# thetengda/OKVIS2-X

Measured on AMD Instinct MI355X. Metric: Gauss-Newton iters/sec on 50-KF/2000-landmark window; ATE vs CPU ref, higher is better.
Workload: dtype f64; 1 GPU; 2048 independent S50 windows (50 KF / 2000 landmarks / 16000 reprojections, 49 IMU factors), DENSE_SCHUR + DOGLEG, all tolerances 0; windows_total=2048, windows_per_gpu=2048, parallelism=replicas x1 (one window batch per GPU, no collective in the loop)

## Files before the change

### okvis2-x_amd/csrc/jv_groups.hpp

```cpp
#pragma once
#include "device_problem.hpp"
#include "okvisgpu_math.hpp"

namespace okg {

static_assert(kLmGroupVisits == 256, "jvGroups runs as 256-thread workgroups of k_lm_backsub_jv");

__device__ __forceinline__ bool jvSelect(const DevProblem& P, int w) {
  const WinState& s = P.st[w];
  return !s.done && s.need_gn && !s.gn_failed;
}

__device__ __forceinline__ void jvAcc(double jc, double jg, double (&a)[3]) {
  a[0] += jc * jc;
  a[1] += jg * jg;
  a[2] += jc * jg;
}

__device__ __forceinline__ void jvGroups(const DevProblem& P, int block) {
  const int gid = (block * 256 + (int)threadIdx.x) >> 4, r = threadIdx.x & 15;
  const double* __restrict__ cF = P.vF;
  const double* __restrict__ yF = P.yF;
  int u = gid, w = 0, nr = 0, nb = 0, ld = 0;
  const double* J = nullptr;
  int off[4] = {-1, -1, -1, -1}, n[4] = {0, 0, 0, 0}, col[4] = {0, 0, 0, 0};
  double* out = nullptr;
  size_t ostride = 0;
  bool live = false;
  __shared__ double sVc[256 / 16][32][2];
  if (gid < P.n_fac) {
    const int f = gid, grp = threadIdx.x >> 4;
    const int fw = gmem(P.imu_win)[f], ffl = gmem(P.imu_flags)[f];
    const int4 blk = gmem(reinterpret_cast<const int4*>(P.imu_blocks))[f];
    const auto gst = gmem(P.st + fw);
    const int sDone = gst->done, sNeed = gst->need_gn, sFail = gst->gn_failed, lcur = gst->lcur;
    const int o0 = blk.x < 0 ? -1 : gmem(P.pose_f)[max(blk.x, 0)], o1 = blk.y < 0 ? -1 : gmem(P.sb_f)[max(blk.y, 0)],
              o2 = blk.z < 0 ? -1 : gmem(P.pose_f)[max(blk.z, 0)], o3 = blk.w < 0 ? -1 : gmem(P.sb_f)[max(blk.w, 0)];
    const int foff = gmem(P.win_foff)[fw];
    const bool fl = (sDone == 0) & (sNeed != 0) & (sFail == 0), act = fl & !(ffl & 2);
    double vcv[2], vgv[2];
#pragma unroll
    for (int h = 0; h < 2; ++h) {
      const int c = r + 16 * h;
      const int q = c < 6 ? 0 : c < 15 ? 1 : c < 21 ? 2 : 3;
      const int cq = c - (q == 0 ? 0 : q == 1 ? 6 : q == 2 ? 15 : 21);
      const int oq = q == 0 ? o0 : q == 1 ? o1 : q == 2 ? o2 : o3;
      const bool ok = act && c < 30 && oq >= 0;
      const size_t i = ok ? (size_t)foff + oq + cq : 0;
      const double sc = gmem(P.sF)[i], cv = gmem(cF)[i], yv = gmem(yF)[i];
      vcv[h] = ok ? sc * cv : 0.0;
      vgv[h] = ok ? -sc * yv : 0.0;
    }
    const auto Jr = gmem(pick2(lcur, P.imu_lin[0], P.imu_lin[1]) + (size_t)(act ? f : 0) * kImuLin + 15 +
                         30 * (size_t)min(r, 14));
    double jr[30];
#pragma unroll
    for (int c = 0; c < 30; ++c) jr[c] = Jr[c];
#pragma unroll
    for (int h = 0; h < 2; ++h) {
      sVc[grp][r + 16 * h][0] = vcv[h];
      sVc[grp][r + 16 * h][1] = vgv[h];
    }
    __builtin_amdgcn_fence(__ATOMIC_RELEASE, "wavefront");
    __builtin_amdgcn_wave_barrier();
    __builtin_amdgcn_fence(__ATOMIC_ACQUIRE, "wavefront");
    double jc0 = 0.0, jg0 = 0.0;
#pragma unroll
    for (int c = 0; c < 30; ++c) {
      jc0 += jr[c] * sVc[grp][c][0];
      jg0 += jr[c] * sVc[grp][c][1];
    }
    double a3[3] = {r < 15 ? jc0 * jc0 : 0.0, r < 15 ? jg0 * jg0 : 0.0, r < 15 ? jc0 * jg0 : 0.0};
#pragma unroll
    for (int k = 0; k < 3; ++k)
#pragma unroll
      for (int m = 8; m > 0; m >>= 1) a3[k] += __shfl_xor(a3[k], m, 64);
    if (fl && r == 0)
      for (int k = 0; k < 3; ++k) P.imu_jv[(size_t)k * P.n_fac + f] = a3[k];
    return;
  }
  if (u < P.n_fac) {
  } else if ((u -= P.n_fac) < P.n_pprior) {
    w = P.pp_win[u];
    if (jvSelect(P, w)) {
      live = true;
      out = P.pp_jv + u;
      ostride = P.n_pprior;
      J = P.pp_lin[P.st[w].lcur] + 42 * (size_t)u + 6;
      nr = 6; ld = 6; nb = 1;
      off[0] = P.pose_f[P.pp_block[u]]; n[0] = 6;
    }
  } else if ((u -= P.n_pprior) < P.n_sbprior) {
    w = P.sbp_win[u];
    if (jvSelect(P, w)) {
      live = true;
      out = P.sbp_jv + u;
      ostride = P.n_sbprior;
      J = P.sbp_lin[P.st[w].lcur] + 90 * (size_t)u + 9;
      nr = 9; ld = 9; nb = 1;
      off[0] = P.sb_f[P.sbp_block[u]]; n[0] = 9;
    }
  } else if ((u -= P.n_sbprior) < P.n_relpose) {
    w = P.rp_win[u];
    if (jvSelect(P, w)) {
      live = true;
      out = P.rp_jv + u;
      ostride = P.n_relpose;
      if (!(P.rp_flags[u] & 2)) {
        J = P.rp_lin[P.st[w].lcur] + kRelPoseLin * (size_t)u + 6;
        nr = 6; ld = 12; nb = 2;
        off[0] = P.pose_f[P.rp_blocks[2 * u]]; off[1] = P.pose_f[P.rp_blocks[2 * u + 1]];
        n[0] = 6; n[1] = 6; col[1] = 6;
// ... 30 lines not shown
```

### okvis2-x_amd/csrc/kernels_backsub.hip

```cpp
#include "device_problem.hpp"
#include "jv_groups.hpp"
#include "launch.hpp"
#include "okvisgpu_math.hpp"

namespace okg {

struct ExtTerm {
  double Je[12], ce[6], ge[6];
};
__device__ __forceinline__ bool loadExtTerm(const DevProblem& P, int o, int w, int xs, const double C_WS[9],
                                            const double p3[3], double w4, const double A[6], ExtTerm& X) {
  if (!(P.obs_flags[o] & 4)) return false;
  const int e = P.cam_pose[P.obs_cam[o]];
  const size_t b = (size_t)P.win_foff[w] + P.pose_f[e];
  extrJacobian(A, C_WS, p3, w4, P.pose[xs] + 7 * (size_t)e, X.Je);
#pragma unroll
  for (int c = 0; c < 6; ++c) {
    const double sc = P.sF[b + c];
    X.ce[c] = sc * P.vF[b + c];
    X.ge[c] = -sc * P.yF[b + c];
  }
  return true;
}

template <bool EXT>
__global__ __launch_bounds__(kLmGroupVisits) void k_lm_backsub_jv(const DevProblem* __restrict__ Pp) {
  const DevProblem& P = *Pp;
  if (!EXT && (int)blockIdx.x >= P.n_lmg) {
    jvGroups(P, (int)blockIdx.x - P.n_lmg);
    return;
  }
  const int t = threadIdx.x;
  const auto gi = gmem(reinterpret_cast<const int4*>(P.lmg_info + kLmgInfo * blockIdx.x));
  const int4 gi0 = gi[0], gi1 = gi[kLmgInfo / 4];
  const int l0 = gi0.x, l1 = gi1.x;
  const int w = gi0.z;
  const int v0 = gi0.y, v1 = gi1.y;
  const int v = v0 + t;
  const bool hasV = v < v1;
  const int vc = hasV ? v : v0;
  const int vLm = gmem(P.visit_lm)[vc], vPose = gmem(P.visit_pose)[vc];
  const int obB = gmem(P.visit_obs_begin)[vc], obE = gmem(P.visit_obs_begin)[vc + 1];
  const auto gst = gmem(P.st + w);
  const int sDone = gst->done, sNeed = gst->need_gn, sFail = gst->gn_failed, sLcur = gst->lcur, sXcur = gst->xcur;
  const bool skip = (sDone != 0) | (sNeed == 0) | (sFail != 0) | (((vLm ^ vPose ^ obB ^ obE) & (vc >> 31)) != 0);
  if (skip) return;
  __shared__ double sQ[3][kLmGroupVisits];
  __shared__ double sC[6][kLmGroupMax];
  const int l = hasV ? vLm : l0;
  const int pose = hasV ? vPose : 0;
  const int ob0 = hasV ? obB : 0, ob1 = hasV ? obE : 0;
  const auto lin = gmem(pick2(sLcur, P.obs_lin[0], P.obs_lin[1]));
  const int64_t S = P.obs_stride;
  const int lfreeI = gmem(P.lm_free)[l], pfI = gmem(P.pose_f)[pose];
  const auto hpp = gmem(pick2(sXcur, P.lm[0], P.lm[1]) + 4 * (size_t)l);
  const auto twp = gmem(pick2(sXcur, P.pose[0], P.pose[1]) + 7 * (size_t)pose);
  const double hp[4] = {hpp[0], hpp[1], hpp[2], hpp[3]};
  double tw[7];
#pragma unroll
  for (int k = 0; k < 7; ++k) tw[k] = (EXT || k < 3) ? twp[k] : 0.0;
  const int fl0 = gmem(P.obs_flags)[obB];
  double A0[6];
#pragma unroll
  for (int k = 0; k < 6; ++k) A0[k] = lin[(2 + k) * S + obB];
  asm volatile("" ::"v"(lfreeI), "v"(pfI), "v"(hp[0]), "v"(hp[1]), "v"(hp[2]), "v"(hp[3]), "v"(tw[0]), "v"(tw[1]),
               "v"(tw[2]), "v"(fl0), "v"(A0[0]), "v"(A0[1]), "v"(A0[2]), "v"(A0[3]), "v"(A0[4]), "v"(A0[5]));
  const int xs = sXcur;
  const int pf = hasV ? pfI : -1;
  const bool lfree = lfreeI != 0;
  double cp[6], gp[6];
  {
    const size_t b = pf >= 0 ? (size_t)P.win_foff[w] + pf : 0;
    const auto sFp = gmem(P.sF + b), vFp = gmem(P.vF + b), yFp = gmem(P.yF + b);
    double sc[6], vv[6], yy[6];
#pragma unroll
    for (int c = 0; c < 6; ++c) {
      sc[c] = sFp[c];
      vv[c] = vFp[c];
      yy[c] = yFp[c];
    }
#pragma unroll
    for (int c = 0; c < 6; ++c) {
      cp[c] = pf >= 0 ? sc[c] * vv[c] : 0.0;
      gp[c] = pf >= 0 ? -sc[c] * yy[c] : 0.0;
    }
  }
  const double w4 = hp[3];
  const double p3[3] = {hp[0] - tw[0] * w4, hp[1] - tw[1] * w4, hp[2] - tw[2] * w4};
  double C_WS[9];
  if (EXT) qrot(qnormalize(Q{tw[3], tw[4], tw[5], tw[6]}), C_WS);

  double q[3] = {0.0, 0.0, 0.0};
  if ((pf >= 0 || EXT) && lfree)
    for (int o = ob0; o < ob1; ++o) {
      double A[6], Jp[12], Jl[6];
      int fl = fl0;
#pragma unroll
      for (int k = 0; k < 6; ++k) A[k] = A0[k];
      if (o != ob0) {
        fl = gmem(P.obs_flags)[o];
#pragma unroll
        for (int k = 0; k < 6; ++k) A[k] = lin[(2 + k) * S + o];
      }
      const bool use = !(fl & 2);
#pragma unroll
      for (int k = 0; k < 6; ++k) A[k] = use ? A[k] : 0.0;
      obsJacobians(A, p3, w4, Jp, Jl);
      ExtTerm X;
      const bool hasE = EXT && loadExtTerm(P, o, w, xs, C_WS, p3, w4, A, X);
#pragma unroll
      for (int r = 0; r < 2; ++r) {
        double jg = 0.0;
#pragma unroll
        for (int c = 0; c < 6; ++c) jg += Jp[r * 6 + c] * gp[c];
        if (hasE)
#pragma unroll
          for (int c = 0; c < 6; ++c) jg += X.Je[r * 6 + c] * X.ge[c];
#pragma unroll
        for (int a = 0; a < 3; ++a) q[a] -= Jl[r * 3 + a] * jg;
      }
    }
#pragma unroll
  for (int a = 0; a < 3; ++a) sQ[a][t] = q[a];
  ldsBarrier();

  double lred[3] = {0.0, 0.0, 0.0};
  if (t < l1 - l0) {
    const int L = l0 + t;
    double c6[6] = {0.0, 0.0, 0.0, 0.0, 0.0, 0.0};
    const int lf = gmem(P.lm_free)[L];
    const int mb = gmem(P.lm_visit_begin)[L] - v0, me = gmem(P.lm_visit_begin)[L + 1] - v0;
    double li[9], s3[3], zz[3], dgv[3], lg[3];
#pragma unroll
    for (int i = 0; i < 9; ++i) li[i] = gmem(P.lm_Linv)[9 * (size_t)L + i];
#pragma unroll
    for (int a = 0; a < 3; ++a) {
      const size_t i = 3 * (size_t)L + a;
      s3[a] = gmem(P.sL)[i];
      zz[a] = gmem(P.lm_zz)[i];
      dgv[a] = gmem(P.diagL)[i];
      lg[a] = gmem(P.lm_g)[i];
    }
    if (lf) {
      double qs[3] = {0.0, 0.0, 0.0};
      for (int m = mb; m < me; ++m)
#pragma unroll
        for (int a = 0; a < 3; ++a) qs[a] += sQ[a][m];
      double u[3];
#pragma unroll
      for (int a = 0; a < 3; ++a) qs[a] *= s3[a];
#pragma unroll
      for (int a = 0; a < 3; ++a) u[a] = zz[a] - (li[a * 3] * qs[0] + li[a * 3 + 1] * qs[1] + li[a * 3 + 2] * qs[2]);
#pragma unroll
      for (int a = 0; a < 3; ++a) {
        double y = 0.0;
#pragma unroll
        for (int c = a; c < 3; ++c) y += li[c * 3 + a] * u[c];
        const size_t i = 3 * (size_t)L + a;
        const double dg = dgv[a];
        gmemw(P.yL)[i] = y;
        const double gn = -dg * y;
        gmemw(P.gnL)[i] = gn;
        const double gr = s3[a] * lg[a] / dg;
        const double vc = gr / dg;
        gmemw(P.dgL)[i] = gr;
        gmemw(P.vL)[i] = vc;
        lred[0] += gr * gr;
        lred[1] += gn * gn;
        lred[2] += gr * gn;
        c6[a] = s3[a] * vc;
        c6[3 + a] = -s3[a] * y;
      }
    }
#pragma unroll
    for (int i = 0; i < 6; ++i) sC[i][t] = c6[i];
  }
  ldsBarrier();

  const int u = hasV ? l - l0 : 0;
  double cl[3], gl[3];
#pragma unroll
  for (int c = 0; c < 3; ++c) {
    cl[c] = sC[c][u];
    gl[c] = sC[3 + c][u];
  }
  double acc[3] = {0.0, 0.0, 0.0};
  for (int o = ob0; o < ob1; ++o) {
    double A[6], Jp[12], Jl[6];
    const bool use = !(gmem(P.obs_flags)[o] & 2);
#pragma unroll
    for (int k = 0; k < 6; ++k) A[k] = lin[(2 + k) * S + o];
#pragma unroll
    for (int k = 0; k < 6; ++k) A[k] = use ? A[k] : 0.0;
    obsJacobians(A, p3, w4, Jp, Jl);
    ExtTerm X;
    const bool hasE = EXT && loadExtTerm(P, o, w, xs, C_WS, p3, w4, A, X);
#pragma unroll
    for (int r = 0; r < 2; ++r) {
      double jc = 0.0, jg = 0.0;
#pragma unroll
      for (int c = 0; c < 6; ++c) {
        jc += Jp[r * 6 + c] * cp[c];
        jg += Jp[r * 6 + c] * gp[c];
      }
      if (hasE)
#pragma unroll
        for (int c = 0; c < 6; ++c) {
          jc += X.Je[r * 6 + c] * X.ce[c];
          jg += X.Je[r * 6 + c] * X.ge[c];
        }
#pragma unroll
      for (int c = 0; c < 3; ++c) {
        jc += Jl[r * 3 + c] * cl[c];
        jg += Jl[r * 3 + c] * gl[c];
      }
      acc[0] += jc * jc;
      acc[1] += jg * jg;
      acc[2] += jc * jg;
    }
  }
  double red[6] = {acc[0], acc[1], acc[2], lred[0], lred[1], lred[2]};
#pragma unroll
  for (int k = 0; k < 6; ++k)
#pragma unroll
    for (int m = 32; m > 0; m >>= 1) red[k] += __shfl_xor(red[k], m, 64);
  __shared__ double sW[kLmGroupVisits / 64][6];
  if ((t & 63) == 0)
#pragma unroll
    for (int k = 0; k < 6; ++k) sW[t >> 6][k] = red[k];
  ldsBarrier();
  if (t < 6) {
    double a = sW[0][t];
#pragma unroll
    for (int wv = 1; wv < kLmGroupVisits / 64; ++wv) a += sW[wv][t];
    gmemw(P.grp_red)[(size_t)blockIdx.x * kGrpRed + t] = a;
  }
}

void launch_lm_backsub(const DevProblem& P, hipStream_t s) {
  if (P.n_xvisit > 0) {
    if (P.n_lmg > 0) hipLaunchKernelGGL(k_lm_backsub_jv<true>, dim3(P.n_lmg), dim3(kLmGroupVisits), 0, s, P.self);
    launch_jv(P, s);
    return;
  }
  const int nb = P.n_lmg + jvBlocks(P);
  if (nb > 0) hipLaunchKernelGGL(k_lm_backsub_jv<false>, dim3(nb), dim3(kLmGroupVisits), 0, s, P.self);
}

}
```

### okvis2-x_amd/csrc/kernels_control.hip

```cpp
#include <cfloat>

#include "block_reduce.hpp"
#include "dev_clock.hpp"
#include "device_problem.hpp"
#include "gradnorm.hpp"
#include "jv_groups.hpp"
#include "launch.hpp"
#include "okvisgpu_math.hpp"

namespace okg {

constexpr int kRBBatch = 256, kRBFew = 1024;

__device__ void finalizeIteration(const DevProblem& P, WinState& s) {
  if (s.done) return;
  if (s.iteration >= P.opt.max_num_iterations) {
    s.done = 1;
    s.termination = 1;
    return;
  }
  if (s.radius <= P.opt.min_radius) {
    s.done = 1;
    s.termination = 0;
  }
// ... 197 lines not shown
  DLCLK(0)
  const int foff = P.win_foff[w], fd = P.win_fdim[w];
  const int l0 = P.win_lm_range[2 * w], l1 = P.win_lm_range[2 * w + 1];
  double gg = 0.0, nn = 0.0, gn = 0.0;
  for (int e = t; e < fd; e += RB) {
    const double a = gmem(P.dgF)[foff + e], b = gmem(P.gnF)[foff + e];
    gg += a * a;
    nn += b * b;
    gn += a * b;
  }
  const int gb = P.win_lmg_range[2 * w], ge = P.win_lmg_range[2 * w + 1];
  for (int g = gb + t; g < ge; g += RB) {
    const auto r = gmem(P.grp_red + (size_t)g * kGrpRed);
    gg += r[3];
    nn += r[4];
    gn += r[5];
  }
  double alpha = s.alpha;
  if (sflagGn) {
    double r6[6];
    double a3[3];
    jvPartials(P, w, t, RB, a3);
    DLCLK(1)
    r6[0] = a3[0]; r6[1] = a3[1]; r6[2] = a3[2]; r6[3] = gg; r6[4] = nn; r6[5] = gn;
    blockSumN<RB, 6>(r6, sh);
    DLCLK(2)
    gg = r6[3];
    nn = r6[4];
    gn = r6[5];
    alpha = gg / r6[0];
    if (t == 0) {
      s.jcc = r6[0];
      s.jgg = r6[1];
      s.jcg = r6[2];
      s.alpha = alpha;
    }
  } else {
    double r3[3] = {gg, nn, gn};
    blockSumN<RB, 3>(r3, sh);
    gg = r3[0];
    nn = r3[1];
    gn = r3[2];
  }
  const double gradient_norm = sqrt(gg), gauss_newton_norm = sqrt(nn);
  const double radius = s.radius;
  double ca, cb;
  int dcase;
  if (gauss_newton_norm <= radius) {
    ca = 0.0; cb = 1.0; dcase = 1;
  } else if (gradient_norm * alpha >= radius) {
    ca = -(radius / gradient_norm); cb = 0.0; dcase = 2;
  } else {
    const double b_dot_a = -alpha * gn;
    const double a_squared_norm = (alpha * gradient_norm) * (alpha * gradient_norm);
    const double b_minus_a_squared_norm = a_squared_norm - 2 * b_dot_a + gauss_newton_norm * gauss_newton_norm;
    const double c = b_dot_a - a_squared_norm;
    const double d = sqrt(c * c + b_minus_a_squared_norm * (radius * radius - a_squared_norm));
    const double beta = (c <= 0) ? (d - c) / b_minus_a_squared_norm : (radius * radius - a_squared_norm) / (d + c);
    ca = -alpha * (1.0 - beta);
    cb = beta;
    dcase = 3;
  }
  const int xs = s.xcur, xd = 1 - s.xcur;
  double sn2 = 0.0, dn2 = 0.0, jr = 0.0;
  const int p0 = P.win_pose_range[2 * w], p1 = P.win_pose_range[2 * w + 1];
  for (int p = p0 + t; p < p1; p += RB) {
    const int pf = gmem(P.pose_f)[p];
    if (pf < 0) continue;
    double dg[6], gn[6], dia[6], sc[6], g[6], x[7];
    for (int c = 0; c < 6; ++c) {
      const size_t i = (size_t)foff + pf + c;
      dg[c] = gmem(P.dgF)[i];
      gn[c] = gmem(P.gnF)[i];
      dia[c] = gmem(P.diagF)[i];
      sc[c] = gmem(P.sF)[i];
      g[c] = gmem(P.gF)[i];
    }
    for (int k = 0; k < 7; ++k) x[k] = gmem(P.pose[xs])[7 * (size_t)p + k];
    double delta[6];
    for (int c = 0; c < 6; ++c) {
      const double v = ca * dg[c] + cb * gn[c];
      dn2 += v * v;
      const double st = v / dia[c];
      gmemw(P.stepF)[(size_t)foff + pf + c] = st;
      delta[c] = st * sc[c];
      jr += delta[c] * g[c];
    }
    const auto y = gmemw(P.pose[xd] + 7 * (size_t)p);
    const Q dq = deltaQ(delta[3], delta[4], delta[5]);
    const Q q = qnormalize(qmul(dq, qnormalize(Q{x[3], x[4], x[5], x[6]})));
    double yv[7] = {x[0] + delta[0], x[1] + delta[1], x[2] + delta[2], q.x, q.y, q.z, q.w};
    for (int k = 0; k < 7; ++k) {
      y[k] = yv[k];
      sn2 += (x[k] - yv[k]) * (x[k] - yv[k]);
    }
  }
  const int b0 = P.win_sb_range[2 * w], b1 = P.win_sb_range[2 * w + 1];
  for (int b = b0 + t; b < b1; b += RB) {
    const int sf = gmem(P.sb_f)[b];
    if (sf < 0) continue;
    const auto y = gmemw(P.sb[xd] + 9 * (size_t)b);
    double dg[9], gn[9], dia[9], sc[9], g[9], x[9];
    for (int c = 0; c < 9; ++c) {
      const size_t i = (size_t)foff + sf + c;
      dg[c] = gmem(P.dgF)[i];
      gn[c] = gmem(P.gnF)[i];
      dia[c] = gmem(P.diagF)[i];
      sc[c] = gmem(P.sF)[i];
      g[c] = gmem(P.gF)[i];
      x[c] = gmem(P.sb[xs])[9 * (size_t)b + c];
    }
    for (int c = 0; c < 9; ++c) {
      const double v = ca * dg[c] + cb * gn[c];
      dn2 += v * v;
      const double st = v / dia[c];
      gmemw(P.stepF)[(size_t)foff + sf + c] = st;
      jr += (st * sc[c]) * g[c];
      const double yv = x[c] + st * sc[c];
      y[c] = yv;
      sn2 += (x[c] - yv) * (x[c] - yv);
    }
  }
  DLCLK(3)
  struct LS { double x[4], dg[3], gn[3], dia[3], sl[3], g[3]; uint8_t f; };
  stridedBatched<RB, (RB >= 1024 ? 1 : 4)>(l0, l1,
                    [&](int l) {
                      LS v;
                      v.f = gmem(P.lm_free)[l];
                      for (int k = 0; k < 4; ++k) v.x[k] = gmem(P.lm[xs])[4 * (size_t)l + k];
                      for (int c = 0; c < 3; ++c) {
                        const size_t i = 3 * (size_t)l + c;
                        v.dg[c] = gmem(P.dgL)[i];
                        v.gn[c] = gmem(P.gnL)[i];
                        v.dia[c] = gmem(P.diagL)[i];
                        v.sl[c] = gmem(P.sL)[i];
                        v.g[c] = gmem(P.gL)[i];
                      }
                      return v;
                    },
                    [&](int l, const LS& v) {
                      if (!v.f) return;
                      const auto y = gmemw(P.lm[xd] + 4 * (size_t)l);
                      for (int c = 0; c < 3; ++c) {
                        const double vv = ca * v.dg[c] + cb * v.gn[c];
                        dn2 += vv * vv;
                        const double st = vv / v.dia[c];
                        gmemw(P.stepL)[3 * (size_t)l + c] = st;
                        jr += (st * v.sl[c]) * v.g[c];
                        const double yv = v.x[c] + st * v.sl[c];
                        y[c] = yv;
                        sn2 += (v.x[c] - yv) * (v.x[c] - yv);
                      }
                      y[3] = v.x[3];
                    });
  DLCLK(4)
  {
    double r3[3] = {sn2, dn2, jr};
    blockSumN<RB, 3>(r3, sh);
    sn2 = r3[0];
    dn2 = r3[1];
    jr = r3[2];
  }
  DLCLK(5)
  DLCLK_END
  if (t != 0) return;
  s.dogleg_step_norm = (dcase == 1) ? gauss_newton_norm : (dcase == 2) ? radius : sqrt(dn2);
  s.step_norm = sqrt(sn2);
  const double jj = (ca * ca) * s.jcc + 2.0 * (ca * cb) * s.jcg + (cb * cb) * s.jgg;
  s.model_cost_change = -(jr + 0.5 * jj);
  if (s.model_cost_change > 0.0) {
    s.step_valid = 1;
    s.consecutive_invalid = 0;
    s.eval_cand = 1;
  } else {
    s.step_valid = 0;
    s.eval_cand = 0;
    if (++s.consecutive_invalid >= P.opt.max_num_consecutive_invalid_steps) {
      s.done = 1;
      s.termination = 2;
      s.iteration -= 1;
      return;
    }
    s.num_unsucc += 1;
    s.mu *= 10.0;
    s.need_gn = 1;
    finalizeIteration(P, s);
  }
}

__global__ __launch_bounds__(256) void k_jv(const DevProblem* __restrict__ Pp) { jvGroups(*Pp, (int)blockIdx.x); }
void launch_jv(const DevProblem& P, hipStream_t s) {
  if (jvBlocks(P) > 0) hipLaunchKernelGGL(k_jv, dim3(jvBlocks(P)), dim3(256), 0, s, P.self);
}
void launch_reduce(const DevProblem& P, int mode, hipStream_t s) {
  if (P.few) hipLaunchKernelGGL(k_reduce<kRBFew>, dim3(P.n_win), dim3(kRBFew), 0, s, P.self, mode);
  else hipLaunchKernelGGL(k_reduce<kRBBatch>, dim3(P.n_win), dim3(kRBBatch), 0, s, P.self, mode);
}
void launch_gradnorm(const DevProblem& P, int lin_mode, hipStream_t s) {
  hipLaunchKernelGGL(k_gradnorm<kRBBatch>, dim3(P.n_win), dim3(kRBBatch), 0, s, P.self, lin_mode);
}
void launch_dogleg(const DevProblem& P, hipStream_t s) {
  if (P.few) hipLaunchKernelGGL(k_dogleg<kRBFew>, dim3(P.n_win), dim3(kRBFew), 0, s, P.self);
  else hipLaunchKernelGGL(k_dogleg<kRBBatch>, dim3(P.n_win), dim3(kRBBatch), 0, s, P.self);
}

__global__ __launch_bounds__(256) void k_select_current(const DevProblem* __restrict__ Pp) {
  const DevProblem& P = *Pp;
  const int w = blockIdx.x;
  if (P.st[w].xcur != 1) return;
  auto copy = [&](const int32_t* range, int stride, const double* src, double* dst) {
    const int64_t b = (int64_t)range[2 * w] * stride, e = (int64_t)range[2 * w + 1] * stride;
    for (int64_t i = b + threadIdx.x; i < e; i += blockDim.x) dst[i] = src[i];
  };
  copy(P.win_pose_range, 7, P.pose[1], P.pose[0]);
  copy(P.win_sb_range, 9, P.sb[1], P.sb[0]);
  copy(P.win_lm_range, 4, P.lm[1], P.lm[0]);
}

void launch_select_current(const DevProblem& P, hipStream_t s) {
  if (P.n_win > 0) hipLaunchKernelGGL(k_select_current, dim3(P.n_win), dim3(256), 0, s, P.self);
}

}
```

### okvis2-x_amd/csrc/launch.hpp

```cpp
#pragma once

#include <hip/hip_runtime.h>

#include "device_problem.hpp"

namespace okg {

void launch_eval(const DevProblem& P, int mode, hipStream_t s);
void launch_eval_few(const DevProblem& P, int mode, hipStream_t s);
void launch_eval_obs(const DevProblem& P, int mode, hipStream_t s);
void launch_eval_imu(const DevProblem& P, int mode, hipStream_t s);
void launch_eval_imu_as_solved(const DevProblem& P, int mode, hipStream_t s);
void launch_imu_append(const DevProblem& P, hipStream_t s);
struct ImuPropagateDev {
  int32_t n;
  double par[7];
  double* poses;
  double* sb;
  const int64_t* t_start;
  const int64_t* t_end;
  const int32_t* sbegin;
  const int64_t* ts;
  const double* ga;
  double* cov;
  double* jac;
  int32_t* steps;
};
void launch_imu_propagate(const ImuPropagateDev& A, hipStream_t s);
void launch_host_gather(const DevProblem& P, int mode, hipStream_t s);
void launch_host_scatter(const DevProblem& P, hipStream_t s);

void launch_lm_blocks(const DevProblem& P, int lin_mode, hipStream_t s);
void launch_imu_hess(const DevProblem& P, int lin_mode, hipStream_t s);
void launch_fgrad(const DevProblem& P, int lin_mode, hipStream_t s);
void launch_lm_prep(const DevProblem& P, hipStream_t s);
void launch_lin_few(const DevProblem& P, hipStream_t s);
void launch_zero_S(const DevProblem& P, hipStream_t s);
void launch_assemble(const DevProblem& P, hipStream_t s);
void launch_lm_backsub(const DevProblem& P, hipStream_t s);
void launch_assemble_gradnorm_few(const DevProblem& P, hipStream_t s);
void launch_assemble_pp(const DevProblem& P, hipStream_t s);
void launch_assemble_sb(const DevProblem& P, hipStream_t s);
void launch_lm_visit(const DevProblem& P, int mode, hipStream_t s);

size_t cholesky_persistent_lds();
size_t cholesky_pipe_lds();
void launch_cholesky(const DevProblem& P, hipStream_t s);
void launch_cholesky_pipe(const DevProblem& P, hipStream_t s, bool split);
void launch_cholesky_split_b(const DevProblem& P, hipStream_t s);

enum ReduceMode { R_COST_INIT = 0, R_COST_CAND = 1, R_JV = 2 };
void launch_reduce(const DevProblem& P, int mode, hipStream_t s);
void launch_jv(const DevProblem& P, hipStream_t s);
void launch_gradnorm(const DevProblem& P, int lin_mode, hipStream_t s);
void launch_dogleg(const DevProblem& P, hipStream_t s);
void launch_select_current(const DevProblem& P, hipStream_t s);

void launch_twopose_compute(const TwoPoseDev& T, hipStream_t s);
void launch_twopose_extr_compute(const TwoPoseExtrDev& T, hipStream_t s);
void launch_twopose_extr_eval(const TwoPoseExtrEvalDev& T, hipStream_t s);

void launch_match_prepare(const MatchDev& M, hipStream_t s);
void launch_match(const MatchDev& M, hipStream_t s);

constexpr uint8_t kLmInitialised = 1, kLmReset = 2, kLmNotInFront = 4;
void launch_update_landmarks(const DevProblem& P, double* quality, uint8_t* flags, double* obs_err, double* dirs,
                             hipStream_t s);

struct CovisWin {
  int32_t lm_begin, n_lm;
  int32_t pose_begin, n_state;
  int32_t word_begin, n_words;
  int32_t state_off, pad_;
  int64_t bits_off;
  int64_t counts_off;
};
constexpr size_t kCovisLdsBudget = 64 * 1024;
constexpr int kCovisTile = 32;
constexpr int kCovisChunk = 32;
constexpr int covisRowStride(int n_words) { return n_words | 1; }
constexpr size_t covisLdsBytes(int n_state, int n_words) { return 8 * (size_t)n_state * (size_t)covisRowStride(n_words); }
constexpr bool covisFitsLds(int n_state, int n_words) { return covisLdsBytes(n_state, n_words) <= kCovisLdsBudget; }
void launch_covis_bits(const DevProblem& P, const CovisWin* wins, int n_wins, const int32_t* word_rec, int n_words_total,
                       const uint8_t* excluded, unsigned long long* bits, hipStream_t s);
void launch_covis_counts(const CovisWin* wins, const int32_t* items0, int n0, size_t lds_bytes, const int32_t* items1,
                         int n1, const unsigned long long* bits, int32_t* counts, int32_t* n_observed, hipStream_t s);

}
```

### okvis2-x_amd/csrc/runtime.cpp

```cpp
#include <hip/hip_runtime.h>

#include <algorithm>
#include <chrono>
#include <cmath>
#include <condition_variable>
#include <cstdio>
#include <cstdlib>
#include <cstring>
#include <functional>
#include <map>
#include <memory>
#include <mutex>
#include <stdexcept>
#include <string>
#include <thread>
#include <vector>

#include "../../include/okvisgpu.h"
#include "device_problem.hpp"
#include "launch.hpp"
#include "loss.hpp"
#include "okvisgpu_math.hpp"
#include "plan.hpp"

// ... 1141 lines not shown
        continue;
      }
      iterStart = nowS();
      if (o->verbose) c->runTimed(c->phaseMs);
      else c->launchIterations(1);
      ++c->replays;
      st = c->readStates();
    }
    c->finish(st, sums);
    return (int)OKVISGPU_OK;
  });
}

static const char* kPhaseNames[OKVISGPU_N_PHASES] = {
    "lm_prep",     "zero_S",   "assemble",   "cholesky",  "lm_backsub", "gn_finalize",
    "jv",          "reduce_jv", "dogleg",   "eval_obs",
    "eval_imu",    "eval_priors", "reduce_cand", "lin_blocks", "gradnorm"};

const char* okvisgpu_phase_name(int32_t i) { return (i >= 0 && i < OKVISGPU_N_PHASES) ? kPhaseNames[i] : ""; }

int okvisgpu_profile_iteration(okvisgpu_ctx* c, double* ms) {
  if (!c || !ms) return OKVISGPU_ERR_INVALID_ARGUMENT;
  if (!c->inSolve) return fail(c, OKVISGPU_ERR_INVALID_ARGUMENT, "profile_iteration needs solve_begin");
  return guarded(c, [&]() {
    for (int i = 0; i < OKVISGPU_N_PHASES; ++i) ms[i] = 0.0;
    c->runTimed(ms);
    c->replays += 1;
    return (int)OKVISGPU_OK;
  });
}

namespace {
enum KernelId {
  K_ASSEMBLE_PP, K_ASSEMBLE_SB, K_CHOLESKY, K_LM_VISIT, K_LM_VISIT_PREP, K_EVAL_IMU, K_EVAL_OBS, K_JV,
  K_FGRAD, K_LM_BACKSUB, K_COUNT
};
const char* kKernelNames[K_COUNT] = {"k_assemble_pp", "k_assemble_sb", "k_cholesky", "k_lm_visit", "k_lm_visit_prep",
                                     "k_eval_imu",    "k_eval_obs",    "k_jv",       "k_fgrad",
                                     "k_lm_backsub_jv"};
const int kKernelBound[K_COUNT] = {0, 0, 1, 0, 0, 0, 0, 0, 0, 0};

double kernelWork(const HostBatch& B, const DevProblem& P, int k) {
  const double d8 = 8.0;
  const double nObs = P.n_obs, nVis = P.n_visit, nLm = P.n_lm, nImu = P.n_imu;
  switch (k) {
    case K_ASSEMBLE_PP: {
      double desc = 0, pairs = 0;
      for (const auto* list : {&B.asm_pp_items, &B.asm_ppl_items})
        for (int it : *list)
          if (it >= 0) { desc += B.pair_cbegin[it + 1] - B.pair_cbegin[it]; pairs += 1; }
      return desc * 16 + (double)P.n_part * 36 * d8 + (double)P.n_seg * (21 + 6) * d8 + pairs * (36 + 12) * d8;
    }
    case K_ASSEMBLE_SB: {
      double desc = 0, entries = 0;
      for (int it : B.asm_sb_items) {
        desc += B.pair_cbegin[it + 1] - B.pair_cbegin[it];
        const int ni = B.fb_kind[B.pair_fi[it]] == 0 ? 6 : 9, nj = B.fb_kind[B.pair_fj[it]] == 0 ? 6 : 9;
        entries += ni * nj;
      }
      return desc * 16 + nImu * kImuLin * d8 + entries * d8;
    }
    case K_CHOLESKY: {
      const double n = 64.0;
      double diag = 0;
      for (int w = 0; w < P.n_win; ++w) diag += B.tileT[w];
      const double panels = (double)B.n_panels, syrk = (double)B.n_band_updates_diag,
                   gemm = (double)(B.n_band_updates - B.n_band_updates_diag);
      return diag * (n * n * n / 3.0 + 2.0 * n * n) + panels * (n * n * n + 4.0 * n * n) +
             syrk * n * n * (n + 1.0) + gemm * 2.0 * n * n * n;
    }
    case K_LM_VISIT:
      return nObs * (kObsLin * d8 + 1) + nVis * (7 * d8 + 16) + (double)P.n_seg * (27 + 6) * d8 +
             (double)B.part_contrib.size() * 4 + (double)P.n_part * 36 * d8 + nLm * 40 * d8;
    case K_LM_VISIT_PREP:
      return nObs * (kObsLin * d8 + 1) + nVis * (7 * d8 + 16) + (double)P.n_seg * 6 * d8 +
             (double)B.part_contrib.size() * 4 + (double)P.n_part * 36 * d8 + nLm * 34 * d8;
    case K_EVAL_IMU: return nImu * (2.0 * kImuState + kImuLin + 2 * 16) * d8 + (double)B.imu_ts.size() * 7 * d8;
    case K_EVAL_OBS: return nObs * (16 + (P.obs_iso ? 8 : 32) + 13 + kObsLin * d8 + 8) + nLm * 4 * d8 + (double)B.pose_f.size() * 7 * d8;
    case K_JV:
      return nImu * (kImuLin + 3) * d8 + (double)P.n_pprior * (42 + 3) * d8 + (double)P.n_sbprior * (90 + 3) * d8 +
             (double)P.n_relpose * (kRelPoseLin + 3) * d8;
    case K_LM_BACKSUB:
      return nObs * (6 * d8 + 1) + nVis * (3 * d8 + 16) + (double)P.n_pose * (7 + 18) * d8 +
             nLm * (4 + 9 + 3 + 3 + 3 + 3 + 12) * d8;
    case K_FGRAD: return (double)P.n_seg * 27 * d8 + nImu * kImuLin * d8 + (double)B.fb_contrib.size() * 16;
  }
  return 0.0;
}
}

int okvisgpu_kernel_count(void) { return K_COUNT; }
const char* okvisgpu_kernel_name(int32_t k) { return (k >= 0 && k < K_COUNT) ? kKernelNames[k] : ""; }

int okvisgpu_time_kernel(okvisgpu_ctx* c, int32_t kernel, int32_t reps, double* avg_ms, double* work,
                         int32_t* bound) {
  if (!c || kernel < 0 || kernel >= K_COUNT || reps < 1) return OKVISGPU_ERR_INVALID_ARGUMENT;
  if (!c->haveProblem) return fail(c, OKVISGPU_ERR_NO_PROBLEM, "no problem set");
  if (c->inSolve) return fail(c, OKVISGPU_ERR_INVALID_ARGUMENT, "time_kernel: call after solve_end");
  return guarded(c, [&]() {
    HIPCHK(hipSetDevice(c->device));
    const DevProblem& P = c->P;
    hipStream_t s = c->stream;
    std::vector<WinState> st = c->readStates();
    for (WinState& w : st) {
      w.done = 0; w.need_gn = 1; w.gn_failed = 0; w.eval_cand = 1; w.accepted = 1; w.step_valid = 2;
      w.z_mu = -1.0;
    }
    HIPCHK(hipMemcpyAsync(P.st, st.data(), sizeof(WinState) * st.size(), hipMemcpyHostToDevice, s));
    std::vector<hipEvent_t> ev;
    size_t used = 0;
    auto event = [&]() {
      if (used == ev.size()) {
        hipEvent_t e;
        HIPCHK(hipEventCreate(&e));
        ev.push_back(e);
      }
      HIPCHK(hipEventRecord(ev[used], s));
      return used++;
    };
    std::vector<std::pair<size_t, size_t>> spans;
    auto timed = [&](auto&& launch) {
      const size_t a = event();
      launch();
      const size_t b = event();
      spans.emplace_back(a, b);
    };
    for (int r = 0; r < reps; ++r) {
      switch (kernel) {
        case K_ASSEMBLE_PP: timed([&] { launch_assemble_pp(P, s); }); break;
        case K_ASSEMBLE_SB: timed([&] { launch_assemble_sb(P, s); }); break;
        case K_LM_VISIT: timed([&] { launch_lm_visit(P, 1, s); }); break;
        case K_LM_VISIT_PREP: timed([&] { launch_lm_visit(P, 2, s); }); break;
        case K_EVAL_IMU:
          if (P.n_imu > 0)
            HIPCHK(hipMemset2DAsync(P.imu_state, sizeof(double) * kImuState, 0, sizeof(double), P.n_imu, s));
          timed([&] { launch_eval_imu_as_solved(P, 1, s); });
          break;
        case K_EVAL_OBS: timed([&] { launch_eval_obs(P, 1, s); }); break;
        case K_JV: timed([&] { launch_jv(P, s); }); break;
        case K_LM_BACKSUB: timed([&] { launch_lm_backsub(P, s); }); break;
        case K_FGRAD: timed([&] { launch_fgrad(P, 1, s); }); break;
        case K_CHOLESKY:
          c->ensureS(s);
          launch_assemble(P, s);
          timed([&] { launch_cholesky(P, s); });
          break;
      }
    }
    HIPCHK(hipGetLastError());
    HIPCHK(hipStreamSynchronize(s));
    double tot = 0.0;
    for (auto& sp : spans) {
      float t = 0.f;
      HIPCHK(hipEventElapsedTime(&t, ev[sp.first], ev[sp.second]));
      tot += t;
    }
    for (auto e : ev) (void)hipEventDestroy(e);
    if (avg_ms) *avg_ms = tot / reps;
    if (work) *work = kernelWork(c->B, P, kernel);
    if (bound) *bound = kKernelBound[kernel];
    return (int)OKVISGPU_OK;
  });
}

int okvisgpu_get_stats(okvisgpu_ctx* c, okvisgpu_problem_stats* st) {
  if (!c || !st) return OKVISGPU_ERR_INVALID_ARGUMENT;
  if (!c->haveProblem) return fail(c, OKVISGPU_ERR_NO_PROBLEM, "no problem set");
// ... 83 lines not shown
    HIPCHK(hipSetDevice(c->device));
    okvisgpu_options o;
    okvisgpu_default_options(&o);
    c->setOptions(o);
    c->resetStates(1e-8);
    c->evalAll(2, c->stream);
    launch_reduce(c->P, R_COST_INIT, c->stream);
    HIPCHK(hipGetLastError());
    auto st = c->readStates();
    if (cost) *cost = st[window].x_cost + st[window].fixed_cost;
    const int h0 = c->B.win_host_range[2 * window], h1 = c->B.win_host_range[2 * window + 1];
    for (int h = h0; h < h1; ++h)
      if (c->hostFail[h - c->P.n_imu]) return fail(c, OKVISGPU_ERR_NUMERICAL, "host_evaluate failed");
    return (int)OKVISGPU_OK;
  });
}

int okvisgpu_linearize_reduce(okvisgpu_ctx* c, int32_t window, int32_t jacobi_scaling, double mu, double* S,
                              double* rhs, double* cost, int32_t* dim_out) {
  if (!c) return OKVISGPU_ERR_INVALID_ARGUMENT;
  if (!c->haveProblem) return fail(c, OKVISGPU_ERR_NO_PROBLEM, "no problem set");
  if (window < 0 || window >= c->P.n_win) return fail(c, OKVISGPU_ERR_INVALID_ARGUMENT, "bad window");
  return guarded(c, [&]() {
    HIPCHK(hipSetDevice(c->device));
    okvisgpu_options o;
    okvisgpu_default_options(&o);
    o.jacobi_scaling = jacobi_scaling;
    c->setOptions(o);
    c->resetStates(mu);
    c->launchInit(2);
    launch_lm_prep(c->P, c->stream);
    launch_assemble(c->P, c->stream);
    HIPCHK(hipGetLastError());
    auto st = c->readStates();
    const int fdim = c->B.win_fdim[window], fpad = c->B.win_fpad[window], dn = c->B.win_fnat[window];
    const int32_t* nat = c->B.f_nat.data() + c->B.win_foff[window];
    if (dim_out) *dim_out = dn;
    if (cost) *cost = st[window].x_cost + st[window].fixed_cost;
    if (S && dn) {
      std::vector<double> full((size_t)fpad * fpad);
      HIPCHK(hipMemcpy(full.data(), c->P.S + c->B.win_soff[window], full.size() * 8, hipMemcpyDeviceToHost));
      for (int r = 0; r < fdim; ++r)
        for (int q = 0; q <= r; ++q) {
          const int a = nat[r], b = nat[q];
          if (a < 0 || b < 0) continue;
          S[(size_t)a * dn + b] = full[(size_t)r * fpad + q];
          S[(size_t)b * dn + a] = full[(size_t)r * fpad + q];
        }
    }
    if (rhs && dn) {
      std::vector<double> v(fdim);
      HIPCHK(hipMemcpy(v.data(), c->P.rhsF + c->B.win_foff[window], sizeof(double) * fdim, hipMemcpyDeviceToHost));
      for (int r = 0; r < fdim; ++r)
        if (nat[r] >= 0) rhs[nat[r]] = v[r];
    }
    if (st[window].gn_failed) return fail(c, OKVISGPU_ERR_NUMERICAL, "landmark block not positive definite");
    return (int)OKVISGPU_OK;
  });
}

int okvisgpu_gauss_newton_step(okvisgpu_ctx* c, int32_t window, const okvisgpu_options* options, double mu,
                               double* y_f, double* y_l, int32_t* dim_out) {
  if (!c) return OKVISGPU_ERR_INVALID_ARGUMENT;
  if (!c->haveProblem) return fail(c, OKVISGPU_ERR_NO_PROBLEM, "no problem set");
  if (c->inSolve) return fail(c, OKVISGPU_ERR_INVALID_ARGUMENT, "gauss_newton_step: call after solve_end");
  if (window < 0 || window >= c->P.n_win) return fail(c, OKVISGPU_ERR_INVALID_ARGUMENT, "bad window");
  return guarded(c, [&]() {
    HIPCHK(hipSetDevice(c->device));
    okvisgpu_options o;
    okvisgpu_default_options(&o);
    if (options) {
      o.jacobi_scaling = options->jacobi_scaling;
      o.cholesky_schedule = options->cholesky_schedule;
      o.min_lm_diagonal = options->min_lm_diagonal;
      o.max_lm_diagonal = options->max_lm_diagonal;
    }
    c->setOptions(o);
    c->resetStates(mu);
    c->ensureS(c->stream);
    c->launchInit(2);
    launch_lm_prep(c->P, c->stream);
    launch_assemble(c->P, c->stream);
    launch_cholesky(c->P, c->stream);
    launch_lm_backsub(c->P, c->stream);
    HIPCHK(hipGetLastError());
    auto st = c->readStates();
    const HostBatch& B = c->B;
    const int fdim = B.win_fdim[window], dn = B.win_fnat[window];
    if (dim_out) *dim_out = dn;
    if (st[window].dev_error)
      throw HipError{"window " + std::to_string(window) + ": the pipelined Cholesky's team wait reached its limit",
                     OKVISGPU_ERR_DEVICE};
    if (st[window].gn_failed) return fail(c, OKVISGPU_ERR_NUMERICAL, "Gauss-Newton step: a block is not positive definite");
    if (y_f && dn) {
      const int32_t* nat = B.f_nat.data() + B.win_foff[window];
      std::vector<double> v(fdim);
      HIPCHK(hipMemcpy(v.data(), c->P.yF + B.win_foff[window], sizeof(double) * fdim, hipMemcpyDeviceToHost));
      for (int r = 0; r < fdim; ++r)
        if (nat[r] >= 0) y_f[nat[r]] = v[r];
    }
    const int nl = c->probs[window]->n_landmarks;
    if (y_l && nl) {
      const int lb = B.lm_base[window];
      const int* perm = &B.lm_perm[lb];
      std::vector<double> v(3 * (size_t)nl);
      HIPCHK(hipMemcpy(v.data(), c->P.yL + 3 * (size_t)lb, sizeof(double) * v.size(), hipMemcpyDeviceToHost));
      for (int k = 0; k < nl; ++k)
        for (int a = 0; a < 3; ++a) y_l[3 * (size_t)perm[k] + a] = B.lm_free[lb + k] ? v[3 * (size_t)k + a] : 0.0;
    }
    return (int)OKVISGPU_OK;
  });
}

int okvisgpu_eval_reprojection(okvisgpu_ctx* c, int32_t window, double* r, double* Jp, double* Jl) {
  if (!c) return OKVISGPU_ERR_INVALID_ARGUMENT;
  if (!c->haveProblem) return fail(c, OKVISGPU_ERR_NO_PROBLEM, "no problem set");
  if (window < 0 || window >= c->P.n_win) return fail(c, OKVISGPU_ERR_INVALID_ARGUMENT, "bad window");
  return guarded(c, [&]() {
    HIPCHK(hipSetDevice(c->device));
    c->resetStates(1e-8);
    launch_eval(c->P, 3, c->stream);
    HIPCHK(hipGetLastError());
    const int64_t S = c->P.obs_stride;
    std::vector<double> lin((size_t)kObsLin * S);
    HIPCHK(hipMemcpyAsync(lin.data(), c->P.obs_lin[0], lin.size() * 8, hipMemcpyDeviceToHost, c->stream));
    HIPCHK(hipStreamSynchronize(c->stream));
    const okvisgpu_problem* pr = c->probs[window];
    const int ob = c->B.obs_base[window], n = pr->n_observations;
    for (int k = 0; k < n; ++k) {
      const int g = ob + k, o = c->B.obs_orig[g];
      if (r) for (int i = 0; i < 2; ++i) r[2 * o + i] = lin[(size_t)i * S + g];
      double A[6], Jpo[12], Jlo[6];
      for (int i = 0; i < 6; ++i) A[i] = lin[(size_t)(2 + i) * S + g];
      const double* hp = &pr->landmarks[4 * pr->obs_landmark[o]];
      const double* tw = &pr->poses[7 * pr->obs_pose[o]];
      const double p3[3] = {hp[0] - tw[0] * hp[3], hp[1] - tw[1] * hp[3], hp[2] - tw[2] * hp[3]};
      obsJacobians(A, p3, hp[3], Jpo, Jlo);
      if (Jp) for (int i = 0; i < 12; ++i) Jp[12 * o + i] = Jpo[i];
      if (Jl) for (int i = 0; i < 6; ++i) Jl[6 * o + i] = Jlo[i];
    }
    return (int)OKVISGPU_OK;
  });
}

int okvisgpu_eval_imu(okvisgpu_ctx* c, int32_t window, int32_t redo_always, double* r, double* J) {
  if (!c) return OKVISGPU_ERR_INVALID_ARGUMENT;
  if (!c->haveProblem) return fail(c, OKVISGPU_ERR_NO_PROBLEM, "no problem set");
  if (window < 0 || window >= c->P.n_win) return fail(c, OKVISGPU_ERR_INVALID_ARGUMENT, "bad window");
  return guarded(c, [&]() {
    HIPCHK(hipSetDevice(c->device));
    okvisgpu_options o;
    okvisgpu_default_options(&o);
    o.redo_propagation_always = redo_always;
    c->setOptions(o);
    c->resetStates(1e-8);
    launch_eval(c->P, 3, c->stream);
    HIPCHK(hipGetLastError());
    const int n = c->probs[window]->n_imu, ib = c->B.imu_base[window];
    std::vector<double> lin((size_t)kImuLin * std::max(1, n));
    if (n) HIPCHK(hipMemcpyAsync(lin.data(), c->P.imu_lin[0] + (size_t)ib * kImuLin, (size_t)kImuLin * n * 8,
                                 hipMemcpyDeviceToHost, c->stream));
    HIPCHK(hipStreamSynchronize(c->stream));
    for (int f = 0; f < n; ++f) {
      if (r) for (int i = 0; i < 15; ++i) r[15 * f + i] = lin[(size_t)f * kImuLin + i];
      if (J) for (int i = 0; i < 450; ++i) J[450 * (size_t)f + i] = lin[(size_t)f * kImuLin + 15 + i];
    }
    c->downloadParams();
// ... 622 lines not shown
```

Measured before the change: 226,000 window-iterations/s.

## Stage per-group observation Jacobian data in LDS and drop unused global stores

New measurement: 228,500 window-iterations/s, median of 6. 1.01x the previous value.

```diff
diff --git a/okvis2-x_amd/csrc/jv_groups.hpp b/okvis2-x_amd/csrc/jv_groups.hpp
--- a/okvis2-x_amd/csrc/jv_groups.hpp
+++ b/okvis2-x_amd/csrc/jv_groups.hpp
@@ -17,7 +17,9 @@
   a[2] += jc * jg;
 }
 
-__device__ __forceinline__ void jvGroups(const DevProblem& P, int block) {
+using JvLds = double[32][2];
+constexpr int kJvLdsGroups = 256 / 16;
+__device__ __forceinline__ void jvGroups(const DevProblem& P, int block, JvLds* sVc) {
   const int gid = (block * 256 + (int)threadIdx.x) >> 4, r = threadIdx.x & 15;
   const double* __restrict__ cF = P.vF;
   const double* __restrict__ yF = P.yF;
@@ -27,7 +29,6 @@
   double* out = nullptr;
   size_t ostride = 0;
   bool live = false;
-  __shared__ double sVc[256 / 16][32][2];
   if (gid < P.n_fac) {
     const int f = gid, grp = threadIdx.x >> 4;
     const int fw = gmem(P.imu_win)[f], ffl = gmem(P.imu_flags)[f];
diff --git a/okvis2-x_amd/csrc/kernels_backsub.hip b/okvis2-x_amd/csrc/kernels_backsub.hip
--- a/okvis2-x_amd/csrc/kernels_backsub.hip
+++ b/okvis2-x_amd/csrc/kernels_backsub.hip
@@ -23,11 +23,26 @@
   return true;
 }
 
+#ifndef OKG_BS_STAGE
+#define OKG_BS_STAGE 1
+#endif
+constexpr int kBsStageObs = 512;
+constexpr int kBsStageDoubles = 6 * kBsStageObs + kBsStageObs / 8;
+static_assert(kBsStageDoubles * sizeof(double) >= sizeof(JvLds) * kJvLdsGroups, "jvGroups' vectors fit in the stage");
+static_assert(kBsStageObs % kLmGroupVisits == 0, "the workgroup fills the stage in whole rounds");
+
+constexpr int kBsStoreY = 1, kBsNoStage = 2;
+
+__shared__ double gBsQ[3][kLmGroupVisits];
+__shared__ double gBsC[6][kLmGroupMax];
+__shared__ double gBsW[kLmGroupVisits / 64][6];
+__shared__ __attribute__((aligned(16))) double gBsStage[kBsStageDoubles];
+
 template <bool EXT>
-__global__ __launch_bounds__(kLmGroupVisits) void k_lm_backsub_jv(const DevProblem* __restrict__ Pp) {
+__global__ __launch_bounds__(kLmGroupVisits) void k_lm_backsub_jv(const DevProblem* __restrict__ Pp, const int flags) {
   const DevProblem& P = *Pp;
   if (!EXT && (int)blockIdx.x >= P.n_lmg) {
-    jvGroups(P, (int)blockIdx.x - P.n_lmg);
+    jvGroups(P, (int)blockIdx.x - P.n_lmg, reinterpret_cast<JvLds*>(gBsStage));
     return;
   }
   const int t = threadIdx.x;
@@ -41,17 +56,38 @@
   const int vc = hasV ? v : v0;
   const int vLm = gmem(P.visit_lm)[vc], vPose = gmem(P.visit_pose)[vc];
   const int obB = gmem(P.visit_obs_begin)[vc], obE = gmem(P.visit_obs_begin)[vc + 1];
+  constexpr bool kStage = OKG_BS_STAGE && !EXT;
+  const int oBegin = kStage ? gmem(P.visit_obs_begin)[v0] : 0;
+  const int nObs = kStage ? gmem(P.visit_obs_begin)[v1] - oBegin : 0;
   const auto gst = gmem(P.st + w);
   const int sDone = gst->done, sNeed = gst->need_gn, sFail = gst->gn_failed, sLcur = gst->lcur, sXcur = gst->xcur;
-  const bool skip = (sDone != 0) | (sNeed == 0) | (sFail != 0) | (((vLm ^ vPose ^ obB ^ obE) & (vc >> 31)) != 0);
+  const bool skip = (sDone != 0) | (sNeed == 0) | (sFail != 0) |
+                    (((vLm ^ vPose ^ obB ^ obE ^ oBegin ^ nObs) & (vc >> 31)) != 0);
   if (skip) return;
-  __shared__ double sQ[3][kLmGroupVisits];
-  __shared__ double sC[6][kLmGroupMax];
+  const bool storeY = (flags & kBsStoreY) != 0;
+  const bool STAGE = kStage && !(flags & kBsNoStage) && nObs <= kBsStageObs;
+  double* const sA = gBsStage;
+  uint8_t* const sFl = reinterpret_cast<uint8_t*>(gBsStage + 6 * kBsStageObs);
+  double (*sQ)[kLmGroupVisits] = gBsQ;
+  double (*sC)[kLmGroupMax] = gBsC;
+  double (*sW)[6] = gBsW;
   const int l = hasV ? vLm : l0;
   const int pose = hasV ? vPose : 0;
   const int ob0 = hasV ? obB : 0, ob1 = hasV ? obE : 0;
   const auto lin = gmem(pick2(sLcur, P.obs_lin[0], P.obs_lin[1]));
   const int64_t S = P.obs_stride;
+  constexpr int kStageRounds = kBsStageObs / kLmGroupVisits;
+  double stg[6][kStageRounds] = {};
+  int flS[kStageRounds] = {};
+  if (STAGE) {
+#pragma unroll
+    for (int j = 0; j < kStageRounds; ++j) {
+      const int o = oBegin + max(min(t + j * kLmGroupVisits, nObs - 1), 0);
+      flS[j] = gmem(P.obs_flags)[o];
+#pragma unroll
+      for (int k = 0; k < 6; ++k) stg[k][j] = lin[(2 + k) * S + o];
+    }
+  }
   const int lfreeI = gmem(P.lm_free)[l], pfI = gmem(P.pose_f)[pose];
   const auto hpp = gmem(pick2(sXcur, P.lm[0], P.lm[1]) + 4 * (size_t)l);
   const auto twp = gmem(pick2(sXcur, P.pose[0], P.pose[1]) + 7 * (size_t)pose);
@@ -59,12 +95,19 @@
   double tw[7];
 #pragma unroll
   for (int k = 0; k < 7; ++k) tw[k] = (EXT || k < 3) ? twp[k] : 0.0;
-  const int fl0 = gmem(P.obs_flags)[obB];
-  double A0[6];
-#pragma unroll
-  for (int k = 0; k < 6; ++k) A0[k] = lin[(2 + k) * S + obB];
-  asm volatile("" ::"v"(lfreeI), "v"(pfI), "v"(hp[0]), "v"(hp[1]), "v"(hp[2]), "v"(hp[3]), "v"(tw[0]), "v"(tw[1]),
-               "v"(tw[2]), "v"(fl0), "v"(A0[0]), "v"(A0[1]), "v"(A0[2]), "v"(A0[3]), "v"(A0[4]), "v"(A0[5]));
+  int fl0 = 0;
+  double A0[6] = {0.0, 0.0, 0.0, 0.0, 0.0, 0.0};
+  if (!STAGE) {
+    fl0 = gmem(P.obs_flags)[obB];
+#pragma unroll
+    for (int k = 0; k < 6; ++k) A0[k] = lin[(2 + k) * S + obB];
+  }
+  if (STAGE)
+    asm volatile("" ::"v"(lfreeI), "v"(pfI), "v"(hp[0]), "v"(hp[1]), "v"(hp[2]), "v"(hp[3]), "v"(tw[0]), "v"(tw[1]),
+                 "v"(tw[2]));
+  else
+    asm volatile("" ::"v"(lfreeI), "v"(pfI), "v"(hp[0]), "v"(hp[1]), "v"(hp[2]), "v"(hp[3]), "v"(tw[0]), "v"(tw[1]),
+                 "v"(tw[2]), "v"(fl0), "v"(A0[0]), "v"(A0[1]), "v"(A0[2]), "v"(A0[3]), "v"(A0[4]), "v"(A0[5]));
   const int xs = sXcur;
   const int pf = hasV ? pfI : -1;
   const bool lfree = lfreeI != 0;
@@ -90,6 +133,16 @@
   double C_WS[9];
   if (EXT) qrot(qnormalize(Q{tw[3], tw[4], tw[5], tw[6]}), C_WS);
 
+  if (STAGE) {
+#pragma unroll
+    for (int j = 0; j < kStageRounds; ++j) {
+      sFl[t + j * kLmGroupVisits] = (uint8_t)flS[j];
+#pragma unroll
+      for (int k = 0; k < 6; ++k) sA[k * kBsStageObs + t + j * kLmGroupVisits] = stg[k][j];
+    }
+    ldsBarrier();
+  }
+
   double q[3] = {0.0, 0.0, 0.0};
   if ((pf >= 0 || EXT) && lfree)
     for (int o = ob0; o < ob1; ++o) {
@@ -97,7 +150,11 @@
       int fl = fl0;
 #pragma unroll
       for (int k = 0; k < 6; ++k) A[k] = A0[k];
-      if (o != ob0) {
+      if (STAGE) {
+        fl = sFl[o - oBegin];
+#pragma unroll
+        for (int k = 0; k < 6; ++k) A[k] = sA[k * kBsStageObs + (o - oBegin)];
+      } else if (o != ob0) {
         fl = gmem(P.obs_flags)[o];
 #pragma unroll
         for (int k = 0; k < 6; ++k) A[k] = lin[(2 + k) * S + o];
@@ -158,13 +215,12 @@
         for (int c = a; c < 3; ++c) y += li[c * 3 + a] * u[c];
         const size_t i = 3 * (size_t)L + a;
         const double dg = dgv[a];
-        gmemw(P.yL)[i] = y;
+        if (storeY) gmemw(P.yL)[i] = y;
         const double gn = -dg * y;
         gmemw(P.gnL)[i] = gn;
         const double gr = s3[a] * lg[a] / dg;
         const double vc = gr / dg;
         gmemw(P.dgL)[i] = gr;
-        gmemw(P.vL)[i] = vc;
         lred[0] += gr * gr;
         lred[1] += gn * gn;
         lred[2] += gr * gn;
@@ -187,9 +243,9 @@
   double acc[3] = {0.0, 0.0, 0.0};
   for (int o = ob0; o < ob1; ++o) {
     double A[6], Jp[12], Jl[6];
-    const bool use = !(gmem(P.obs_flags)[o] & 2);
-#pragma unroll
-    for (int k = 0; k < 6; ++k) A[k] = lin[(2 + k) * S + o];
+    const bool use = !((STAGE ? sFl[o - oBegin] : gmem(P.obs_flags)[o]) & 2);
+#pragma unroll
+    for (int k = 0; k < 6; ++k) A[k] = STAGE ? sA[k * kBsStageObs + (o - oBegin)] : lin[(2 + k) * S + o];
 #pragma unroll
     for (int k = 0; k < 6; ++k) A[k] = use ? A[k] : 0.0;
     obsJacobians(A, p3, w4, Jp, Jl);
@@ -224,7 +280,6 @@
   for (int k = 0; k < 6; ++k)
 #pragma unroll
     for (int m = 32; m > 0; m >>= 1) red[k] += __shfl_xor(red[k], m, 64);
-  __shared__ double sW[kLmGroupVisits / 64][6];
   if ((t & 63) == 0)
 #pragma unroll
     for (int k = 0; k < 6; ++k) sW[t >> 6][k] = red[k];
@@ -237,14 +292,16 @@
   }
 }
 
-void launch_lm_backsub(const DevProblem& P, hipStream_t s) {
+void launch_lm_backsub(const DevProblem& P, hipStream_t s, bool storeY) {
+  const int flags = (storeY ? kBsStoreY : 0) | (P.few ? kBsNoStage : 0);
   if (P.n_xvisit > 0) {
-    if (P.n_lmg > 0) hipLaunchKernelGGL(k_lm_backsub_jv<true>, dim3(P.n_lmg), dim3(kLmGroupVisits), 0, s, P.self);
+    if (P.n_lmg > 0)
+      hipLaunchKernelGGL(k_lm_backsub_jv<true>, dim3(P.n_lmg), dim3(kLmGroupVisits), 0, s, P.self, flags);
     launch_jv(P, s);
     return;
   }
   const int nb = P.n_lmg + jvBlocks(P);
-  if (nb > 0) hipLaunchKernelGGL(k_lm_backsub_jv<false>, dim3(nb), dim3(kLmGroupVisits), 0, s, P.self);
+  if (nb > 0) hipLaunchKernelGGL(k_lm_backsub_jv<false>, dim3(nb), dim3(kLmGroupVisits), 0, s, P.self, flags);
 }
 
 }
diff --git a/okvis2-x_amd/csrc/kernels_control.hip b/okvis2-x_amd/csrc/kernels_control.hip
--- a/okvis2-x_amd/csrc/kernels_control.hip
+++ b/okvis2-x_amd/csrc/kernels_control.hip
@@ -303,7 +303,6 @@
       const double v = ca * dg[c] + cb * gn[c];
       dn2 += v * v;
       const double st = v / dia[c];
-      gmemw(P.stepF)[(size_t)foff + pf + c] = st;
       delta[c] = st * sc[c];
       jr += delta[c] * g[c];
     }
@@ -335,7 +334,6 @@
       const double v = ca * dg[c] + cb * gn[c];
       dn2 += v * v;
       const double st = v / dia[c];
-      gmemw(P.stepF)[(size_t)foff + sf + c] = st;
       jr += (st * sc[c]) * g[c];
       const double yv = x[c] + st * sc[c];
       y[c] = yv;
@@ -366,7 +364,6 @@
                         const double vv = ca * v.dg[c] + cb * v.gn[c];
                         dn2 += vv * vv;
                         const double st = vv / v.dia[c];
-                        gmemw(P.stepL)[3 * (size_t)l + c] = st;
                         jr += (st * v.sl[c]) * v.g[c];
                         const double yv = v.x[c] + st * v.sl[c];
                         y[c] = yv;
@@ -409,7 +406,10 @@
   }
 }
 
-__global__ __launch_bounds__(256) void k_jv(const DevProblem* __restrict__ Pp) { jvGroups(*Pp, (int)blockIdx.x); }
+__global__ __launch_bounds__(256) void k_jv(const DevProblem* __restrict__ Pp) {
+  __shared__ double sVc[kJvLdsGroups][32][2];
+  jvGroups(*Pp, (int)blockIdx.x, sVc);
+}
 void launch_jv(const DevProblem& P, hipStream_t s) {
   if (jvBlocks(P) > 0) hipLaunchKernelGGL(k_jv, dim3(jvBlocks(P)), dim3(256), 0, s, P.self);
 }
diff --git a/okvis2-x_amd/csrc/launch.hpp b/okvis2-x_amd/csrc/launch.hpp
--- a/okvis2-x_amd/csrc/launch.hpp
+++ b/okvis2-x_amd/csrc/launch.hpp
@@ -37,7 +37,7 @@
 void launch_lin_few(const DevProblem& P, hipStream_t s);
 void launch_zero_S(const DevProblem& P, hipStream_t s);
 void launch_assemble(const DevProblem& P, hipStream_t s);
-void launch_lm_backsub(const DevProblem& P, hipStream_t s);
+void launch_lm_backsub(const DevProblem& P, hipStream_t s, bool storeY = false);
 void launch_assemble_gradnorm_few(const DevProblem& P, hipStream_t s);
 void launch_assemble_pp(const DevProblem& P, hipStream_t s);
 void launch_assemble_sb(const DevProblem& P, hipStream_t s);
diff --git a/okvis2-x_amd/csrc/runtime.cpp b/okvis2-x_amd/csrc/runtime.cpp
--- a/okvis2-x_amd/csrc/runtime.cpp
+++ b/okvis2-x_amd/csrc/runtime.cpp
@@ -1247,7 +1247,7 @@
              (double)P.n_relpose * (kRelPoseLin + 3) * d8;
     case K_LM_BACKSUB:
       return nObs * (6 * d8 + 1) + nVis * (3 * d8 + 16) + (double)P.n_pose * (7 + 18) * d8 +
-             nLm * (4 + 9 + 3 + 3 + 3 + 3 + 12) * d8;
+             nLm * (4 + 9 + 3 + 3 + 3 + 3 + 6) * d8 + (double)P.n_lmg * kGrpRed * d8;
     case K_FGRAD: return (double)P.n_seg * 27 * d8 + nImu * kImuLin * d8 + (double)B.fb_contrib.size() * 16;
   }
   return 0.0;
@@ -1497,7 +1497,7 @@
     launch_lm_prep(c->P, c->stream);
     launch_assemble(c->P, c->stream);
     launch_cholesky(c->P, c->stream);
-    launch_lm_backsub(c->P, c->stream);
+    launch_lm_backsub(c->P, c->stream, true);
     HIPCHK(hipGetLastError());
     auto st = c->readStates();
     const HostBatch& B = c->B;
```
